# ceselder/pacman-marl-2025

Measured on AMD Instinct MI355X. Metric: env-steps/s (4-agent smallCapture), higher is better.
Workload: dtype u32; 1 GPU; smallCapture.lay 2v2, 16384 envs/GPU, gymPacMan tick (self_play), length 300, auto-reset, uniform random actions (Philox seed 1234), 4 observations/env-tick; envs_per_gpu=16384, layout=smallCapture, obs_dtype=float32, obs_bytes_per_elem=4, parallelism=env-sharded x1, no data-path collective

## Files before the change

### pacman-marl-2025_amd/csrc/pmx_actor.hip

```cpp
#pragma clang fp contract(fast)
#include <hip/hip_runtime.h>
#include <hip/hip_bf16.h>
#include <stdint.h>

#include "../../include/pmx.h"

namespace {

typedef __attribute__((ext_vector_type(8))) short bf16x8;
typedef __attribute__((ext_vector_type(4))) short bf16x4;
typedef __attribute__((ext_vector_type(4))) float f32x4;
typedef __attribute__((ext_vector_type(2))) float f32x2;
typedef __attribute__((ext_vector_type(2))) __bf16 bf16x2_t;

constexpr int NLAYER = 8;
constexpr int GUARD = 1;
constexpr int FRAG_PER_LAYER = 2 * 9 * 64 * 8;
constexpr size_t PACK_FWD = 0;
constexpr size_t PACK_BWD = PACK_FWD + (size_t)NLAYER * FRAG_PER_LAYER * 2;
constexpr size_t PACK_BIAS = PACK_BWD + (size_t)NLAYER * FRAG_PER_LAYER * 2;
constexpr size_t PACK_GNW = PACK_BIAS + NLAYER * 32 * 4;
constexpr size_t PACK_GNB = PACK_GNW + NLAYER * 32 * 4;
constexpr size_t PACK_BYTES = PACK_GNB + NLAYER * 32 * 4;
static_assert(PACK_BYTES == PMX_ACTOR_PACK_BYTES, "include/pmx.h and pmx_actor.hip disagree on the pack size");
constexpr int GRAD_W = 0;
constexpr int GRAD_B = GRAD_W + NLAYER * 36 * 256;
constexpr int GRAD_GNW = GRAD_B + NLAYER * 32;
constexpr int GRAD_GNB = GRAD_GNW + NLAYER * 32;
constexpr int GRAD_FLOATS = GRAD_GNB + NLAYER * 32;
constexpr int W_PART_ROWS = 128;
static_assert(GRAD_FLOATS == PMX_ACTOR_GRAD_FLOATS, "include/pmx.h and pmx_actor.hip disagree on the gradient size");

__host__ __device__ constexpr int map_positions(int nt, int wp) { return GUARD + wp + 32 * ((nt + 1) / 2) + wp + 3; }

__device__ __forceinline__ int map_off(int pos, int chunk) { return pos * 64 + (chunk << 4); }

__device__ __forceinline__ uint32_t pack2(float a, float b)
{
    f32x2 f = {a, b};
    return __builtin_bit_cast(uint32_t, __builtin_convertvector(f, bf16x2_t));
}
__device__ __forceinline__ float lo_f(uint32_t u) { return __uint_as_float(u << 16); }
__device__ __forceinline__ float hi_f(uint32_t u) { return __uint_as_float(u & 0xFFFF0000u); }

__device__ __forceinline__ f32x2 fma2(f32x2 a, f32x2 b, f32x2 c) { return __builtin_elementwise_fma(a, b, c); }
__device__ __forceinline__ f32x2 splat2(float v) { return f32x2{v, v}; }
__device__ __forceinline__ f32x2 unpack2(uint32_t u) { return f32x2{lo_f(u), hi_f(u)}; }
__device__ __forceinline__ f32x2 phi_cdf2(f32x2 z, f32x2 &e)
{
    const f32x2 den = {fmaf(0.3275911f * 0.70710678118654752f, fabsf(z.x), 1.0f), fmaf(0.3275911f * 0.70710678118654752f, fabsf(z.y), 1.0f)};
    const f32x2 t = {__builtin_amdgcn_rcpf(den.x), __builtin_amdgcn_rcpf(den.y)};
    f32x2 poly = fma2(t, splat2(0.5f * 1.061405429f), splat2(0.5f * -1.453152027f));
    poly = fma2(poly, t, splat2(0.5f * 1.421413741f));
    poly = fma2(poly, t, splat2(0.5f * -0.284496736f));
    poly = fma2(poly, t, splat2(0.5f * 0.254829592f));
    poly *= t;
    const f32x2 arg = (z * z) * splat2(-0.5f * 1.4426950408889634f);
    e = f32x2{__builtin_amdgcn_exp2f(arg.x), __builtin_amdgcn_exp2f(arg.y)};
    const f32x2 half_tail = poly * e, rest = splat2(1.0f) - half_tail;
    return f32x2{z.x >= 0.0f ? rest.x : half_tail.x, z.y >= 0.0f ? rest.y : half_tail.y};
}
__device__ __forceinline__ uint2 gelu_quad(uint2 h2, uint2 r2, float mean, float rstd, const float (&gw)[4], const float (&gb)[4], float vm)
{
    f32x2 v[2];
#pragma unroll
    for (int k = 0; k < 2; ++k) {
        const f32x2 hv = unpack2(k ? h2.y : h2.x), rv = unpack2(k ? r2.y : r2.x);
        const f32x2 z = rv + fma2((hv - splat2(mean)) * splat2(rstd), f32x2{gw[2 * k], gw[2 * k + 1]}, f32x2{gb[2 * k], gb[2 * k + 1]});
        f32x2 e;
        v[k] = z * phi_cdf2(z, e) * splat2(vm);
    }
    return uint2{pack2(v[0].x, v[0].y), pack2(v[1].x, v[1].y)};
}
__device__ __forceinline__ uint2 dgelu_quad(uint2 dy, uint2 h2, uint2 x2, float rstd, float nmr, const f32x2 (&gw2)[2], const f32x2 (&gb2)[2],
                                            f32x2 (&dgw2)[2], f32x2 (&dgb2)[2])
{
    f32x2 xh[2], dzf[2];
#pragma unroll
    for (int k = 0; k < 2; ++k) {
        const f32x2 hv = unpack2(k ? h2.y : h2.x), xv = unpack2(k ? x2.y : x2.x), d = unpack2(k ? dy.y : dy.x);
        xh[k] = fma2(hv, splat2(rstd), splat2(nmr));
        const f32x2 z = xv + fma2(xh[k], gw2[k], gb2[k]);
        f32x2 e;
        const f32x2 phi = phi_cdf2(z, e);
        dzf[k] = d * fma2(z * splat2(0.3989422804014327f), e, phi);
    }
    uint2 dzq = {pack2(dzf[0].x, dzf[0].y), pack2(dzf[1].x, dzf[1].y)};
    asm volatile("" : "+v"(dzq.x), "+v"(dzq.y));
#pragma unroll
    for (int k = 0; k < 2; ++k) {
        const f32x2 dzr = unpack2(k ? dzq.y : dzq.x);
        dgb2[k] += dzr;
        dgw2[k] = fma2(dzr, xh[k], dgw2[k]);
    }
    return dzq;
}

template <typename T> __device__ __forceinline__ float in_to_f(T v);
template <> __device__ __forceinline__ float in_to_f<uint8_t>(uint8_t v) { return (float)v; }
template <> __device__ __forceinline__ float in_to_f<float>(float v) { return v; }
template <> __device__ __forceinline__ float in_to_f<__hip_bfloat16>(__hip_bfloat16 v) { return __bfloat162float(v); }

__device__ __forceinline__ void wave_lds_fence()
{
    __builtin_amdgcn_fence(__ATOMIC_ACQ_REL, "wavefront");
    __builtin_amdgcn_wave_barrier();
}

template <int CTRL> __device__ __forceinline__ float dpp_f(float v)
{
    return __builtin_bit_cast(float, __builtin_amdgcn_update_dpp(0, __builtin_bit_cast(int, v), CTRL, 0xF, 0xF, true));
}
__device__ __forceinline__ float row16_sum(float v)
{
    v += dpp_f<0xB1>(v);
    v += dpp_f<0x4E>(v);
    v += dpp_f<0x141>(v);
    v += dpp_f<0x140>(v);
    return v;
}
__device__ __forceinline__ float group_sum(float v)
{
    v = row16_sum(v);
    float a = v, b = v;
    asm volatile("s_nop 1\n\tv_permlane16_swap_b32 %0, %1" : "+v"(a), "+v"(b));
    return a + b;
}
__device__ __forceinline__ float pos_sum(float v) { return row16_sum(v); }

struct Geom {
    int H, W, WP, HW, MP;
};

template <typename IN_T>
__device__ __forceinline__ void load_obs(const IN_T *__restrict__ obs, char *map, const Geom &G, int lane)
{
    for (int i = lane; i < G.HW; i += 64) {
        const int row = i / G.W, col = i - row * G.W;
        const int pos = (row + 1) * G.WP + col + 1 + GUARD;
        float v[8];
#pragma unroll
        for (int c = 0; c < 8; ++c) v[c] = in_to_f<IN_T>(obs[c * G.HW + i]);
        uint4 w = {pack2(v[0], v[1]), pack2(v[2], v[3]), pack2(v[4], v[5]), pack2(v[6], v[7])};
        *reinterpret_cast<uint4 *>(map + map_off(pos, 0)) = w;
        const uint4 z = {0, 0, 0, 0};
#pragma unroll
        for (int ch = 1; ch < 4; ++ch) *reinterpret_cast<uint4 *>(map + map_off(pos, ch)) = z;
    }
}

__device__ __forceinline__ void load_frags(bf16x8 (&A)[2][9], const short *__restrict__ frag, int lane)
{
#pragma unroll
    for (int m = 0; m < 2; ++m)
#pragma unroll
        for (int k = 0; k < 9; ++k) A[m][k] = *reinterpret_cast<const bf16x8 *>(frag + ((m * 9 + k) * 64 + lane) * 8);
}

__device__ __forceinline__ void conv_tile(const char *lane_base, const bf16x8 (&A)[2][9], int centre, int wp64, f32x4 &a0, f32x4 &a1)
{
    a0 = f32x4{0.f, 0.f, 0.f, 0.f};
    a1 = f32x4{0.f, 0.f, 0.f, 0.f};
#pragma unroll
    for (int ky = 0; ky < 3; ++ky) {
        const char *row = lane_base + (centre + (ky - 1) * wp64 - 64);
#pragma unroll
        for (int kx = 0; kx < 3; ++kx) {
            const bf16x8 b = *reinterpret_cast<const bf16x8 *>(row + kx * 64);
            a0 = __builtin_amdgcn_mfma_f32_16x16x32_bf16(A[0][ky * 3 + kx], b, a0, 0, 0, 0);
            a1 = __builtin_amdgcn_mfma_f32_16x16x32_bf16(A[1][ky * 3 + kx], b, a1, 0, 0, 0);
        }
    }
}

__device__ __forceinline__ size_t dump_index(size_t sample, int NT, int t, int m, int lane) { return ((sample * NT + t) * 2 + m) * 64 + lane; }

template <int NT, typename IN_T, bool SAVE>
__global__ __launch_bounds__(256, 2) void pmx_actor_fwd_kernel(const IN_T *__restrict__ obs, const char *__restrict__ pack,
                                                              uint2 *__restrict__ feat, uint2 *__restrict__ hsave,
                                                              uint2 *__restrict__ ysave, float *__restrict__ stats,
                                                              uint2 *__restrict__ rtmp, int B, int H, int W, float eps)
{
    extern __shared__ __attribute__((aligned(16))) char smem[];
    const int lane = threadIdx.x & 63, wave = threadIdx.x >> 6;
    const int p = lane & 15, g = lane >> 4;
    Geom G;
    G.H = H, G.W = W, G.WP = W + 2, G.HW = H * W, G.MP = map_positions(NT, W + 2);
    char *map = smem + (size_t)wave * G.MP * 64;
    for (int i = lane; i < G.MP * 4; i += 64) reinterpret_cast<uint4 *>(map)[i] = uint4{0, 0, 0, 0};
    __shared__ int cell_tab[NT * 16];
    for (int i = threadIdx.x; i < NT * 16; i += 256) {
        const int q = G.WP + i, row = q / G.WP, col = q - row * G.WP;
        cell_tab[i] = (col >= 1 && col <= W && row <= H) ? (row - 1) * W + (col - 1) : -1;
    }
    __syncthreads();
    uint32_t vmask = 0;
#pragma unroll
    for (int t = 0; t < NT; ++t) {
        const int q = G.WP + 16 * t + p, row = q / G.WP, col = q - row * G.WP;
        if (col >= 1 && col <= W && row <= H) vmask |= 1u << t;
    }
    const short *fw = reinterpret_cast<const short *>(pack + PACK_FWD);
    const float *biasp = reinterpret_cast<const float *>(pack + PACK_BIAS);
    const float *gnwp = reinterpret_cast<const float *>(pack + PACK_GNW);
    const float *gnbp = reinterpret_cast<const float *>(pack + PACK_GNB);
    const float inv_n = 1.0f / (float)(8 * G.HW);

    for (int s = blockIdx.x * 4 + wave; s < B; s += gridDim.x * 4) {
        wave_lds_fence();
        load_obs<IN_T>(obs + (size_t)s * 8 * G.HW, map, G, lane);
        wave_lds_fence();
        const short *fws = fw;
        asm volatile("" : "+s"(fws));
        bf16x8 A[2][9];
        load_frags(A, fws, lane);
#pragma unroll 1
        for (int li = 0; li < NLAYER; ++li) {
            int l = li;
            asm volatile("" : "+s"(l));
            const bool has_gn = l >= 2;
            const bool res_on = l >= 3 && (l & 1);
            int WPv = G.WP, pq = p + GUARD;
            uint32_t vmk = vmask;
            asm volatile("" : "+s"(WPv));
            asm volatile("" : "+v"(pq), "+v"(vmk));
            uint2 *ydst = SAVE ? ysave + dump_index((size_t)l * B + s, NT, 0, 0, lane)
                               : rtmp + dump_index((size_t)blockIdx.x * 4 + wave, NT, 0, 0, lane);
            const uint2 *rsrc = SAVE ? ysave + dump_index((size_t)(l >= 2 ? l - 2 : 0) * B + s, NT, 0, 0, lane) : ydst;
            const bool write_y = SAVE || (l & 1);
            float bias[2][4];
#pragma unroll
            for (int m = 0; m < 2; ++m)
#pragma unroll
                for (int r = 0; r < 4; ++r) bias[m][r] = biasp[l * 32 + 16 * m + 4 * g + r];
            uint2 hp[NT][2];
            float s1[2] = {0.f, 0.f}, s2[2] = {0.f, 0.f};
            const char *rbase = map + pq * 64 + g * 16;
            char *wbase = map + pq * 64 + g * 8;
#pragma unroll
            for (int t = 0; t < NT; ++t) {
                f32x4 a[2];
                conv_tile(rbase, A, (WPv + 16 * t) * 64, WPv * 64, a[0], a[1]);
                const float vm = ((vmk >> t) & 1) ? 1.0f : 0.0f;
#pragma unroll
                for (int m = 0; m < 2; ++m) {
                    float v[4];
#pragma unroll
                    for (int r = 0; r < 4; ++r) v[r] = (a[m][r] + bias[m][r]) * vm;
                    uint2 h2 = {pack2(v[0], v[1]), pack2(v[2], v[3])};
                    asm volatile("" : "+v"(h2.x), "+v"(h2.y));
                    hp[t][m] = h2;
                    const float h0 = lo_f(h2.x), h1 = hi_f(h2.x), h2f = lo_f(h2.y), h3 = hi_f(h2.y);
                    s1[m] += (h0 + h1) + (h2f + h3);
                    s2[m] += fmaf(h0, h0, h1 * h1) + fmaf(h2f, h2f, h3 * h3);
                    if (SAVE) hsave[dump_index((size_t)l * B + s, NT, t, m, lane)] = h2;
                }
                __builtin_amdgcn_sched_barrier(0);
            }
            load_frags(A, fws + (size_t)(l + 1 < NLAYER ? l + 1 : l) * FRAG_PER_LAYER, lane);
            constexpr int RD = 2;
            float gw[2][4], gb[2][4];
            uint2 rres[NT][2];
#pragma unroll
            for (int t = 0; t < NT; ++t) rres[t][0] = rres[t][1] = uint2{0u, 0u};
            if (res_on) {
#pragma unroll
                for (int t = 0; t < RD; ++t)
#pragma unroll
                    for (int m = 0; m < 2; ++m) rres[t][m] = rsrc[(t * 2 + m) * 64];
            }
            float mean[2], rstd[2];
#pragma unroll
            for (int m = 0; m < 2; ++m) {
                const float a1 = group_sum(s1[m]) * inv_n, a2 = group_sum(s2[m]) * inv_n;
                mean[m] = has_gn ? a1 : 0.0f;
                rstd[m] = has_gn ? __builtin_amdgcn_rsqf(fmaxf(a2 - a1 * a1, 0.0f) + eps) : 1.0f;
            }
            if (SAVE && p == 0 && (g & 1) == 0) {
#pragma unroll
                for (int m = 0; m < 2; ++m) {
                    float *st = stats + (((size_t)l * B + s) * 4 + 2 * m + (g >> 1)) * 2;
                    st[0] = mean[m], st[1] = rstd[m];
                }
            }
#pragma unroll
            for (int m = 0; m < 2; ++m)
#pragma unroll
                for (int r = 0; r < 4; ++r) gw[m][r] = gnwp[l * 32 + 16 * m + 4 * g + r], gb[m][r] = gnbp[l * 32 + 16 * m + 4 * g + r];
            wave_lds_fence();
#pragma unroll
            for (int t = 0; t < NT; ++t) {
                const float vm = ((vmk >> t) & 1) ? 1.0f : 0.0f;
                if (t + RD < NT && res_on) {
#pragma unroll
                    for (int m = 0; m < 2; ++m) rres[t + RD][m] = rsrc[((t + RD) * 2 + m) * 64];
                }
#pragma unroll
                for (int m = 0; m < 2; ++m) {
                    const uint2 y2 = gelu_quad(hp[t][m], rres[t][m], mean[m], rstd[m], gw[m], gb[m], vm);
                    *reinterpret_cast<uint2 *>(wbase + (WPv + 16 * t) * 64 + m * 32) = y2;
                    if (write_y) ydst[(t * 2 + m) * 64] = y2;
                    if (l == NLAYER - 1) {
                        const int ci = cell_tab[16 * t + p];
                        if (ci >= 0) feat[((size_t)s * G.HW + ci) * 8 + 4 * m + g] = y2;
                    }
                    __builtin_amdgcn_sched_barrier(0);
// ... 410 lines not shown
#pragma unroll
        for (int w = 0; w < 4; ++w) v += reinterpret_cast<const float *>(smem + (size_t)w * (G.MP * 64 + NLAYER * 96 * 4) + (size_t)G.MP * 64)[i];
        accpart[(size_t)blockIdx.x * (NLAYER * 96) + i] = v;
    }
}

template <int NT, int WS>
__global__ __launch_bounds__(256, 2) void pmx_actor_bwd_data_split_kernel(const char *__restrict__ pack, const uint2 *__restrict__ dfeat,
                                                                         const uint2 *__restrict__ hsave, const uint2 *__restrict__ ysave,
                                                                         const float *__restrict__ stats, bf16x8 *__restrict__ dasave,
                                                                         uint2 *__restrict__ sktmp, float *__restrict__ accpart, int B,
                                                                         int H, int W)
{
    constexpr int NTW = (NT + WS - 1) / WS, SPB = 4 / WS, KS = (NT + 1) / 2;
    constexpr bool XG_LATE = NT > 16;
    extern __shared__ __attribute__((aligned(16))) char smem[];
    const int lane = threadIdx.x & 63, wave = threadIdx.x >> 6;
    const int p = lane & 15, g = lane >> 4;
    Geom G;
    G.H = H, G.W = W, G.WP = W + 2, G.HW = H * W, G.MP = map_positions(NT, W + 2);
    const int sub = __builtin_amdgcn_readfirstlane(wave / WS), wq = __builtin_amdgcn_readfirstlane(wave % WS);
    char *map = smem + (size_t)sub * G.MP * 64;
    float *acc = reinterpret_cast<float *>(smem + (size_t)SPB * G.MP * 64) + wave * (NLAYER * 96);
    float *xs = reinterpret_cast<float *>(smem + (size_t)SPB * G.MP * 64) + 4 * (NLAYER * 96) + sub * (WS * 8);
    for (int i = threadIdx.x; i < SPB * G.MP * 4; i += 256) reinterpret_cast<uint4 *>(smem)[i] = uint4{0, 0, 0, 0};
    for (int i = lane; i < NLAYER * 96; i += 64) acc[i] = 0.0f;
    const int t0 = __builtin_amdgcn_readfirstlane(wq * NTW);
    uint32_t vmask = 0;
#pragma unroll
    for (int tl = 0; tl < NTW; ++tl) {
        const int q = G.WP + 16 * (t0 + tl) + p, row = q / G.WP, col = q - row * G.WP;
        if (t0 + tl < NT && col >= 1 && col <= W && row <= H) vmask |= 1u << tl;
    }
    const short *bw = reinterpret_cast<const short *>(pack + PACK_BWD);
    const float *gnwp = reinterpret_cast<const float *>(pack + PACK_GNW);
    const float *gnbp = reinterpret_cast<const float *>(pack + PACK_GNB);
    const float inv_n = 1.0f / (float)(8 * G.HW);
    const int tr_row = (lane & 15) >> 2, tr_pc = lane & 3;

    for (int s0 = blockIdx.x * SPB; s0 < B; s0 += gridDim.x * SPB) {
        const bool live = s0 + sub < B;
        const int s = live ? s0 + sub : B - 1;
        uint2 dv[NTW][2];
        uint2 *skp = sktmp + dump_index((size_t)blockIdx.x * SPB + sub, NT, 0, 0, lane);
        {
            int WPo = G.WP;
            asm volatile("" : "+s"(WPo));
#pragma unroll
            for (int tl = 0; tl < NTW; ++tl) {
                const int q = WPo + 16 * (t0 + tl) + p, row = q / WPo, col = q - row * WPo;
                const bool valid = (vmask >> tl) & 1;
#pragma unroll
                for (int m = 0; m < 2; ++m) {
                    dv[tl][m] = uint2{0, 0};
                    if (valid) dv[tl][m] = dfeat[((size_t)s * G.HW + (row - 1) * W + (col - 1)) * 8 + 4 * m + g];
                }
            }
        }
        uint2 hp[NTW][2], xg[NTW][2];
        float gw[2][4], gb[2][4], mean[2], rstd[2], nmr[2];
        auto load_layer_inputs = [&](int ln) {
            const bool res_n = ln >= 3 && (ln & 1);
            const int lres = ln >= 2 ? ln - 2 : 0;
#pragma unroll
            for (int m = 0; m < 2; ++m) {
#pragma unroll
                for (int r = 0; r < 4; ++r) gw[m][r] = gnwp[ln * 32 + 16 * m + 4 * g + r], gb[m][r] = gnbp[ln * 32 + 16 * m + 4 * g + r];
                const float *st = stats + (((size_t)ln * B + s) * 4 + 2 * m + (g >> 1)) * 2;
                mean[m] = st[0], rstd[m] = st[1];
                nmr[m] = -mean[m] * rstd[m];
            }
#pragma unroll
            for (int tl = 0; tl < NTW; ++tl)
#pragma unroll
                for (int m = 0; m < 2; ++m) {
                    hp[tl][m] = uint2{0u, 0u};
                    if (!XG_LATE) xg[tl][m] = uint2{0u, 0u};
                    if (t0 + tl < NT) {
                        hp[tl][m] = hsave[dump_index((size_t)ln * B + s, NT, t0 + tl, m, lane)];
                        if (!XG_LATE && res_n) xg[tl][m] = ysave[dump_index((size_t)lres * B + s, NT, t0 + tl, m, lane)];
                    }
                }
        };
        load_layer_inputs(NLAYER - 1);
#pragma unroll 1
        for (int li = NLAYER - 1; li >= 0; --li) {
            int l = __builtin_amdgcn_readfirstlane(li);
            asm volatile("" : "+s"(l));
            const bool has_gn = l >= 2, has_res = l >= 3 && (l & 1), adds_skip = l >= 2 && !(l & 1);
            const float gn_on = has_gn ? 1.0f : 0.0f;
            int WPv = G.WP, pq = p + GUARD;
            uint32_t vmk = vmask;
            asm volatile("" : "+s"(WPv));
            asm volatile("" : "+v"(pq), "+v"(vmk));
            if (XG_LATE) {
#pragma unroll
                for (int tl = 0; tl < NTW; ++tl)
#pragma unroll
                    for (int m = 0; m < 2; ++m) {
                        xg[tl][m] = uint2{0u, 0u};
                        if (has_res && t0 + tl < NT) xg[tl][m] = ysave[dump_index((size_t)(l - 2) * B + s, NT, t0 + tl, m, lane)];
                    }
            }
            float S1[2], S2[2];
            float dgw[2][4], dgb[2][4];
            f32x2 dgw2[2][2], dgb2[2][2], gw2[2][2], gb2[2][2];
#pragma unroll
            for (int m = 0; m < 2; ++m)
#pragma unroll
                for (int k = 0; k < 2; ++k) {
                    dgw2[m][k] = dgb2[m][k] = f32x2{0.0f, 0.0f};
                    gw2[m][k] = f32x2{gw[m][2 * k], gw[m][2 * k + 1]}, gb2[m][k] = f32x2{gb[m][2 * k], gb[m][2 * k + 1]};
                }
#pragma unroll
            for (int tl = 0; tl < NTW; ++tl) {
                if (t0 + tl < NT) {
#pragma unroll
                    for (int m = 0; m < 2; ++m) {
                        dv[tl][m] = dgelu_quad(dv[tl][m], hp[tl][m], xg[tl][m], rstd[m], nmr[m], gw2[m], gb2[m], dgw2[m], dgb2[m]);
                        __builtin_amdgcn_sched_barrier(0);
                    }
                }
            }
#pragma unroll
            for (int m = 0; m < 2; ++m)
#pragma unroll
                for (int k = 0; k < 2; ++k)
                    dgw[m][2 * k] = dgw2[m][k].x, dgw[m][2 * k + 1] = dgw2[m][k].y, dgb[m][2 * k] = dgb2[m][k].x, dgb[m][2 * k + 1] = dgb2[m][k].y;
            if (has_res) {
#pragma unroll
                for (int tl = 0; tl < NTW; ++tl)
                    if (t0 + tl < NT) {
#pragma unroll
                        for (int m = 0; m < 2; ++m) skp[((t0 + tl) * 2 + m) * 64] = dv[tl][m];
                    }
            }
#pragma unroll
            for (int m = 0; m < 2; ++m) {
                float t1 = 0.f, t2 = 0.f;
#pragma unroll
                for (int r = 0; r < 4; ++r) t1 = fmaf(gw[m][r], dgb[m][r], t1), t2 = fmaf(gw[m][r], dgw[m][r], t2);
                const float a1 = group_sum(t1), a2 = group_sum(t2);
                if (p == 0 && (g & 1) == 0) {
                    xs[(wq * 4 + 2 * m + (g >> 1)) * 2] = a1;
                    xs[(wq * 4 + 2 * m + (g >> 1)) * 2 + 1] = a2;
                }
            }
            const short *bws = bw + (size_t)l * FRAG_PER_LAYER;
            asm volatile("" : "+s"(bws));
            bf16x8 A[2][9];
            load_frags(A, bws, lane);
            __syncthreads();
#pragma unroll
            for (int m = 0; m < 2; ++m) {
                const int grp = 2 * m + (g >> 1);
                float a1 = 0.f, a2 = 0.f;
#pragma unroll
                for (int w = 0; w < WS; ++w) { a1 += xs[(w * 4 + grp) * 2]; a2 += xs[(w * 4 + grp) * 2 + 1]; }
                S1[m] = a1 * inv_n * gn_on, S2[m] = a2 * inv_n * gn_on;
            }
            float Ad[2][4], K2[2], K3[2];
#pragma unroll
            for (int m = 0; m < 2; ++m) {
                K2[m] = -rstd[m] * rstd[m] * S2[m];
                K3[m] = -mean[m] * K2[m] - rstd[m] * S1[m];
#pragma unroll
                for (int r = 0; r < 4; ++r) Ad[m][r] = rstd[m] * gw[m][r];
            }
            float dbias[2][4];
#pragma unroll
            for (int m = 0; m < 2; ++m)
#pragma unroll
                for (int r = 0; r < 4; ++r) dbias[m][r] = 0.0f;
            char *wbase = map + pq * 64 + g * 8;
#pragma unroll
            for (int tl = 0; tl < NTW; ++tl) {
                const int t = t0 + tl;
                if (t < NT) {
                    const float vm = ((vmk >> tl) & 1) ? 1.0f : 0.0f;
#pragma unroll
                    for (int m = 0; m < 2; ++m) {
                        const uint2 h2 = hp[tl][m];
                        const float hv[4] = {lo_f(h2.x), hi_f(h2.x), lo_f(h2.y), hi_f(h2.y)};
                        const float dzr[4] = {lo_f(dv[tl][m].x), hi_f(dv[tl][m].x), lo_f(dv[tl][m].y), hi_f(dv[tl][m].y)};
                        float dh[4];
#pragma unroll
                        for (int r = 0; r < 4; ++r) dh[r] = vm * fmaf(Ad[m][r], dzr[r], fmaf(hv[r], K2[m], K3[m]));
                        const uint2 d2 = {pack2(dh[0], dh[1]), pack2(dh[2], dh[3])};
                        dbias[m][0] += lo_f(d2.x), dbias[m][1] += hi_f(d2.x), dbias[m][2] += lo_f(d2.y), dbias[m][3] += hi_f(d2.y);
                        *reinterpret_cast<uint2 *>(wbase + (WPv + 16 * t) * 64 + m * 32) = d2;
                    }
                }
                __builtin_amdgcn_sched_barrier(0);
            }
            uint2 skip[NTW][2];
#pragma unroll
            for (int tl = 0; tl < NTW; ++tl) {
                skip[tl][0] = skip[tl][1] = uint2{0u, 0u};
                if (adds_skip && t0 + tl < NT) {
#pragma unroll
                    for (int m = 0; m < 2; ++m) skip[tl][m] = skp[((t0 + tl) * 2 + m) * 64];
                }
            }
            load_layer_inputs(l > 0 ? l - 1 : 0);
            if (live) {
#pragma unroll
                for (int m = 0; m < 2; ++m)
#pragma unroll
                    for (int r = 0; r < 4; ++r) {
                        const float b = pos_sum(dbias[m][r]), w = pos_sum(dgw[m][r]), c = pos_sum(dgb[m][r]);
                        if (p == 0) {
                            float *a3 = acc + l * 96 + 16 * m + 4 * g + r;
                            a3[0] += b, a3[32] += w, a3[64] += c;
                        }
                    }
            }
            __syncthreads();
            {
                bf16x8 *dst = dasave + (((size_t)l * B + s) * KS * 2) * 64 + lane;
                const char *tbase = map + (8 * g + tr_row + GUARD) * 64 + tr_pc * 8;
#pragma unroll 1
                for (int ks = wq; ks < KS; ks += WS) {
#pragma unroll
                    for (int mo = 0; mo < 2; ++mo) {
                        const char *o0 = tbase + (WPv + 32 * ks) * 64 + mo * 32;
                        const bf16x4 lo = __builtin_amdgcn_ds_read_tr16_b64_v4i16((bf16x4 __attribute__((address_space(3))) *)(o0));
                        const bf16x4 hi = __builtin_amdgcn_ds_read_tr16_b64_v4i16((bf16x4 __attribute__((address_space(3))) *)(o0 + 256));
                        dst[(ks * 2 + mo) * 64] = bf16x8{lo[0], lo[1], lo[2], lo[3], hi[0], hi[1], hi[2], hi[3]};
                    }
                }
            }
            if (l > 0) {
#pragma unroll
                for (int tl = 0; tl < NTW; ++tl) {
                    const int t = t0 + tl;
                    if (t < NT) {
                        f32x4 a[2];
                        conv_tile(map + pq * 64 + g * 16, A, (WPv + 16 * t) * 64, WPv * 64, a[0], a[1]);
                        const float vm = ((vmk >> tl) & 1) ? 1.0f : 0.0f;
#pragma unroll
                        for (int m = 0; m < 2; ++m) {
                            const uint32_t sx = skip[tl][m].x, sy = skip[tl][m].y;
                            const float v0 = (lo_f(sx) + a[m][0]) * vm, v1 = (hi_f(sx) + a[m][1]) * vm;
                            const float v2 = (lo_f(sy) + a[m][2]) * vm, v3 = (hi_f(sy) + a[m][3]) * vm;
                            uint2 nx = {pack2(v0, v1), pack2(v2, v3)};
                            asm volatile("" : "+v"(nx.x), "+v"(nx.y));
                            dv[tl][m] = nx;
                        }
                    }
                    __builtin_amdgcn_sched_barrier(0);
                }
            }
        }
        __syncthreads();
    }
    __syncthreads();
    for (int i = threadIdx.x; i < NLAYER * 96; i += 256) {
        const float *a0 = reinterpret_cast<const float *>(smem + (size_t)SPB * G.MP * 64);
        accpart[(size_t)blockIdx.x * (NLAYER * 96) + i] = (a0[i] + a0[NLAYER * 96 + i]) + (a0[2 * NLAYER * 96 + i] + a0[3 * NLAYER * 96 + i]);
    }
}

__global__ __launch_bounds__(256) void pmx_actor_sum_acc_kernel(const float *__restrict__ accpart, int n_rows, float *__restrict__ grad)
{
    __shared__ float part[8][33];
    const int c = threadIdx.x & 31, sl = threadIdx.x >> 5;
    const int i = blockIdx.x * 32 + c;
    float acc[4] = {0.f, 0.f, 0.f, 0.f};
    int r = sl;
    for (; r + 24 < n_rows; r += 32) {
#pragma unroll
        for (int k = 0; k < 4; ++k) acc[k] += accpart[(size_t)(r + 8 * k) * (NLAYER * 96) + i];
    }
    for (; r < n_rows; r += 8) acc[0] += accpart[(size_t)r * (NLAYER * 96) + i];
    part[sl][c] = (acc[0] + acc[1]) + (acc[2] + acc[3]);
    __syncthreads();
    if (sl == 0) {
        float t = 0.f;
#pragma unroll
        for (int k = 0; k < 8; ++k) t += part[k][c];
        const int l = i / 96, j = i - l * 96, kind = j >> 5, ch = j & 31;
        grad[(kind == 0 ? GRAD_B : kind == 1 ? GRAD_GNW : GRAD_GNB) + l * 32 + ch] = t;
    }
}

__global__ __launch_bounds__(256) void pmx_actor_sum_w_kernel(const float *__restrict__ wpart, int n_rows, float *__restrict__ grad)
{
    __shared__ float part[8][33];
    const int c = threadIdx.x & 31, sl = threadIdx.x >> 5;
    const int i = blockIdx.x * 32 + c;
    constexpr size_t ROW = (size_t)NLAYER * 36 * 256;
    float acc = 0.f;
    for (int r = sl; r < n_rows; r += 8) acc += wpart[(size_t)r * ROW + i];
    part[sl][c] = acc;
    __syncthreads();
    if (sl == 0) {
        float t = 0.f;
#pragma unroll
        for (int k = 0; k < 8; ++k) t += part[k][c];
        grad[GRAD_W + i] = t;
    }
}

template <int NT, typename IN_T>
__global__ __launch_bounds__(256, 2) void pmx_actor_bwd_weight_kernel(const IN_T *__restrict__ obs, const uint2 *__restrict__ ysave,
                                                                     const bf16x8 *__restrict__ dasave, float *__restrict__ grad,
                                                                     int B, int H, int W, int per_wave)
{
    extern __shared__ __attribute__((aligned(16))) char smem[];
    const int lane = threadIdx.x & 63, wave = threadIdx.x >> 6;
    const int p = lane & 15, g = lane >> 4;
    const int l = blockIdx.y;
    Geom G;
    G.H = H, G.W = W, G.WP = W + 2, G.HW = H * W, G.MP = map_positions(NT, W + 2);
    constexpr int KS = (NT + 1) / 2;
    char *mapB = smem + (size_t)wave * G.MP * 64;
    for (int i = lane; i < G.MP * 4; i += 64) reinterpret_cast<uint4 *>(mapB)[i] = uint4{0, 0, 0, 0};
    const int tr_row = (lane & 15) >> 2, tr_pc = lane & 3;
    f32x4 accw[36];
#pragma unroll
    for (int i = 0; i < 36; ++i) accw[i] = f32x4{0.f, 0.f, 0.f, 0.f};
    const int s_begin = (blockIdx.x * 4 + wave) * per_wave;
    const int s_end = s_begin + per_wave < B ? s_begin + per_wave : B;
    for (int s = s_begin; s < s_end; ++s) {
        int WPv = G.WP, pq = p + GUARD;
        asm volatile("" : "+s"(WPv));
        asm volatile("" : "+v"(pq));
        wave_lds_fence();
        if (l == 0) {
            load_obs<IN_T>(obs + (size_t)s * 8 * G.HW, mapB, G, lane);
        } else {
            uint2 xin[NT][2];
#pragma unroll
            for (int t = 0; t < NT; ++t)
#pragma unroll
                for (int m = 0; m < 2; ++m) xin[t][m] = ysave[dump_index((size_t)(l - 1) * B + s, NT, t, m, lane)];
#pragma unroll
            for (int t = 0; t < NT; ++t)
#pragma unroll
                for (int m = 0; m < 2; ++m)
                    *reinterpret_cast<uint2 *>(mapB + pq * 64 + g * 8 + (WPv + 16 * t) * 64 + m * 32) = xin[t][m];
        }
        wave_lds_fence();
        const bf16x8 *asrc = dasave + (((size_t)l * B + s) * KS * 2) * 64 + lane;
#pragma unroll 1
        for (int ks = 0; ks < KS; ++ks) {
            const bf16x8 Ad0 = asrc[(ks * 2 + 0) * 64], Ad1 = asrc[(ks * 2 + 1) * 64];
            const char *tbase = mapB + (8 * g + tr_row + GUARD) * 64 + tr_pc * 8 + (WPv + 32 * ks) * 64;
#pragma unroll
            for (int ky = 0; ky < 3; ++ky)
#pragma unroll
                for (int kx = 0; kx < 3; ++kx) {
                    const char *tx = tbase + ((ky - 1) * WPv + (kx - 1)) * 64;
#pragma unroll
                    for (int ni = 0; ni < 2; ++ni) {
                        const bf16x4 lo = __builtin_amdgcn_ds_read_tr16_b64_v4i16((bf16x4 __attribute__((address_space(3))) *)(tx + ni * 32));
                        const bf16x4 hi = __builtin_amdgcn_ds_read_tr16_b64_v4i16((bf16x4 __attribute__((address_space(3))) *)(tx + ni * 32 + 256));
                        const bf16x8 Bx = bf16x8{lo[0], lo[1], lo[2], lo[3], hi[0], hi[1], hi[2], hi[3]};
                        accw[(0 * 2 + ni) * 9 + ky * 3 + kx] = __builtin_amdgcn_mfma_f32_16x16x32_bf16(Ad0, Bx, accw[(0 * 2 + ni) * 9 + ky * 3 + kx], 0, 0, 0);
                        accw[(1 * 2 + ni) * 9 + ky * 3 + kx] = __builtin_amdgcn_mfma_f32_16x16x32_bf16(Ad1, Bx, accw[(1 * 2 + ni) * 9 + ky * 3 + kx], 0, 0, 0);
                    }
                }
        }
    }
    __syncthreads();
    float *red = reinterpret_cast<float *>(smem);
    constexpr int PER_ROUND = 9;
#pragma unroll
    for (int round = 0; round < 4; ++round) {
#pragma unroll
        for (int i = 0; i < PER_ROUND; ++i)
            *reinterpret_cast<f32x4 *>(red + ((size_t)(wave * PER_ROUND + i) * 64 + lane) * 4) = accw[round * PER_ROUND + i];
        __syncthreads();
        for (int i = threadIdx.x; i < PER_ROUND * 64; i += 256) {
            f32x4 v = *reinterpret_cast<const f32x4 *>(red + (size_t)i * 4);
#pragma unroll
            for (int w = 1; w < 4; ++w) {
                const f32x4 u = *reinterpret_cast<const f32x4 *>(red + ((size_t)w * PER_ROUND * 64 + i) * 4);
                v[0] += u[0], v[1] += u[1], v[2] += u[2], v[3] += u[3];
            }
            float *dst = grad + ((size_t)blockIdx.x * NLAYER * 36 + (size_t)l * 36 + round * PER_ROUND) * 256 + (size_t)i * 4;
            *reinterpret_cast<f32x4 *>(dst) = v;
        }
        __syncthreads();
    }
}

template <int NT, typename IN_T>
__global__ __launch_bounds__(256, 2) void pmx_actor_bwd_weight_split_kernel(const IN_T *__restrict__ obs, const uint2 *__restrict__ ysave,
                                                                           const bf16x8 *__restrict__ dasave, float *__restrict__ wpart,
                                                                           int B, int H, int W, int per_pair)
{
    constexpr int KS = (NT + 1) / 2, NTH = (NT + 1) / 2;
    extern __shared__ __attribute__((aligned(16))) char smem[];
    const int lane = threadIdx.x & 63, wave = threadIdx.x >> 6;
    const int p = lane & 15, g = lane >> 4;
    const int l = blockIdx.y;
    const int sub = __builtin_amdgcn_readfirstlane(wave >> 1), ni = __builtin_amdgcn_readfirstlane(wave & 1);
    Geom G;
    G.H = H, G.W = W, G.WP = W + 2, G.HW = H * W, G.MP = map_positions(NT, W + 2);
    char *mapB = smem + (size_t)sub * G.MP * 64;
    for (int i = threadIdx.x; i < 2 * G.MP * 4; i += 256) reinterpret_cast<uint4 *>(smem)[i] = uint4{0, 0, 0, 0};
    const int tr_row = (lane & 15) >> 2, tr_pc = lane & 3;
    f32x4 accw[18];
#pragma unroll
    for (int i = 0; i < 18; ++i) accw[i] = f32x4{0.f, 0.f, 0.f, 0.f};
    const int pair = blockIdx.x * 2 + sub;
    const int s_begin = pair * per_pair;
    uint2 xin[NTH][2];
    auto fetch = [&](int s) {
#pragma unroll
        for (int tl = 0; tl < NTH; ++tl)
#pragma unroll
            for (int m = 0; m < 2; ++m) {
                const int t = ni * NTH + tl;
                xin[tl][m] = uint2{0u, 0u};
                if (t < NT) xin[tl][m] = ysave[dump_index((size_t)(l - 1) * B + s, NT, t, m, lane)];
            }
    };
    if (l > 0 && s_begin < B) fetch(s_begin);
    for (int i = 0; i < per_pair; ++i) {
        const int s = s_begin + i;
        const bool live = s < B;
        int WPv = G.WP, pq = p + GUARD;
        asm volatile("" : "+s"(WPv));
        asm volatile("" : "+v"(pq));
        __syncthreads();
        if (live) {
            if (l == 0) {
                load_obs_block<IN_T>(obs + (size_t)s * 8 * G.HW, mapB, G, ni * 64 + lane, 128);
            } else {
#pragma unroll
                for (int tl = 0; tl < NTH; ++tl) {
                    const int t = ni * NTH + tl;
                    if (t < NT) {
#pragma unroll
                        for (int m = 0; m < 2; ++m)
                            *reinterpret_cast<uint2 *>(mapB + pq * 64 + g * 8 + (WPv + 16 * t) * 64 + m * 32) = xin[tl][m];
                    }
                }
            }
        }
        __syncthreads();
        if (l > 0 && i + 1 < per_pair && s + 1 < B) fetch(s + 1);
        if (live) {
            const bf16x8 *asrc = dasave + (((size_t)l * B + s) * KS * 2) * 64 + lane;
            bf16x8 An0 = asrc[0], An1 = asrc[64];
#pragma unroll 2
            for (int ks = 0; ks < KS; ++ks) {
                const bf16x8 Ad0 = An0, Ad1 = An1;
                if (ks + 1 < KS) { An0 = asrc[((ks + 1) * 2 + 0) * 64]; An1 = asrc[((ks + 1) * 2 + 1) * 64]; }
                const char *tbase = mapB + (8 * g + tr_row + GUARD) * 64 + tr_pc * 8 + (WPv + 32 * ks) * 64 + ni * 32;
#pragma unroll
                for (int ky = 0; ky < 3; ++ky)
#pragma unroll
                    for (int kx = 0; kx < 3; ++kx) {
                        const char *tx = tbase + ((ky - 1) * WPv + (kx - 1)) * 64;
                        const bf16x4 lo = __builtin_amdgcn_ds_read_tr16_b64_v4i16((bf16x4 __attribute__((address_space(3))) *)(tx));
                        const bf16x4 hi = __builtin_amdgcn_ds_read_tr16_b64_v4i16((bf16x4 __attribute__((address_space(3))) *)(tx + 256));
                        const bf16x8 Bx = bf16x8{lo[0], lo[1], lo[2], lo[3], hi[0], hi[1], hi[2], hi[3]};
                        accw[ky * 3 + kx] = __builtin_amdgcn_mfma_f32_16x16x32_bf16(Ad0, Bx, accw[ky * 3 + kx], 0, 0, 0);
                        accw[9 + ky * 3 + kx] = __builtin_amdgcn_mfma_f32_16x16x32_bf16(Ad1, Bx, accw[9 + ky * 3 + kx], 0, 0, 0);
                    }
            }
        }
    }
    float *dst = wpart + ((size_t)pair * NLAYER * 36 + (size_t)l * 36) * 256 + (size_t)lane * 4;
#pragma unroll
    for (int mo = 0; mo < 2; ++mo)
#pragma unroll
        for (int k = 0; k < 9; ++k) *reinterpret_cast<f32x4 *>(dst + (size_t)((mo * 2 + ni) * 9 + k) * 256) = accw[mo * 9 + k];
}

struct PackArgs {
    const float *w[NLAYER], *b[NLAYER], *gw[NLAYER], *gb[NLAYER];
    int cin[NLAYER], cout[NLAYER];
};

__global__ __launch_bounds__(256) void pmx_actor_pack_kernel(PackArgs a, char *__restrict__ pack)
{
    const int l = blockIdx.y;
    short *fw = reinterpret_cast<short *>(pack + PACK_FWD) + (size_t)l * FRAG_PER_LAYER;
    short *bw = reinterpret_cast<short *>(pack + PACK_BWD) + (size_t)l * FRAG_PER_LAYER;
    const int cin = a.cin[l], cout = a.cout[l];
    for (int i = blockIdx.x * 256 + threadIdx.x; i < FRAG_PER_LAYER; i += gridDim.x * 256) {
        const int j = i & 7, lane = (i >> 3) & 63, k = (i >> 9) % 9, m = i / (512 * 9);
        const int row = 16 * m + (lane & 15), kk = 8 * (lane >> 4) + j;
        float vf = 0.f, vb = 0.f;
        if (row < cout && kk < cin) vf = a.w[l][((size_t)row * cin + kk) * 9 + k];
        if (row < cin && kk < cout) vb = a.w[l][((size_t)kk * cin + row) * 9 + (8 - k)];
        fw[i] = (short)(pack2(vf, 0.f) & 0xFFFF);
        bw[i] = (short)(pack2(vb, 0.f) & 0xFFFF);
    }
    if (blockIdx.x == 0 && threadIdx.x < 32) {
        const int c = threadIdx.x;
        reinterpret_cast<float *>(pack + PACK_BIAS)[l * 32 + c] = c < cout ? a.b[l][c] : 0.f;
        reinterpret_cast<float *>(pack + PACK_GNW)[l * 32 + c] = a.gw[l] ? a.gw[l][c] : 1.f;
        reinterpret_cast<float *>(pack + PACK_GNB)[l * 32 + c] = a.gb[l] ? a.gb[l][c] : 0.f;
    }
}

struct UnpackArgs {
    float *w[NLAYER], *b[NLAYER], *gw[NLAYER], *gb[NLAYER];
    int cin[NLAYER], cout[NLAYER];
};

__global__ __launch_bounds__(256) void pmx_actor_unpack_kernel(UnpackArgs a, const float *__restrict__ grad)
{
    const int l = blockIdx.y;
    const int cin = a.cin[l], cout = a.cout[l];
    for (int i = blockIdx.x * 256 + threadIdx.x; i < 36 * 256; i += gridDim.x * 256) {
        const int r = i & 3, lane = (i >> 2) & 63, tile = i >> 8;
        const int k = tile % 9, ni = (tile / 9) & 1, mo = tile / 18;
        const int co = 16 * mo + 4 * (lane >> 4) + r, ci = 16 * ni + (lane & 15);
        if (co < cout && ci < cin) a.w[l][((size_t)co * cin + ci) * 9 + k] = grad[GRAD_W + (size_t)l * 36 * 256 + i];
    }
    if (blockIdx.x == 0 && threadIdx.x < 32) {
        const int c = threadIdx.x;
        if (c < cout) a.b[l][c] = grad[GRAD_B + l * 32 + c];
        if (a.gw[l]) a.gw[l][c] = grad[GRAD_GNW + l * 32 + c];
        if (a.gb[l]) a.gb[l][c] = grad[GRAD_GNB + l * 32 + c];
    }
}

int tiles_for(int H, int W) { return (H * (W + 2) + 15) / 16; }

}

static const int kCin[NLAYER] = {8, 16, 32, 32, 32, 32, 32, 32};
static const int kCout[NLAYER] = {16, 32, 32, 32, 32, 32, 32, 32};

static bool tiles_supported(int nt) { return nt == 10 || nt == 11 || nt == 28; }
constexpr bool large_board(int nt) { return nt > 16; }

extern "C" int pmx_actor_supported(int32_t H, int32_t W)
{
    if (H < 1 || W < 1 || H > PMX_MAX_DIM || W > PMX_MAX_DIM) return 0;
    return tiles_supported(tiles_for(H, W)) ? 1 : 0;
}

extern "C" int pmx_actor_sizes(int32_t H, int32_t W, int64_t B, int64_t *save_bytes, int64_t *scratch_bytes, int64_t *infer_scratch_bytes)
{
    if (!pmx_actor_supported(H, W) || B < 0) return PMX_ERR_UNSUPPORTED;
    const int64_t dump = (int64_t)tiles_for(H, W) * 1024;
    if (save_bytes) *save_bytes = B * (8 * dump + 8 * dump + 8 * 4 * 2 * 4);
    const int64_t infer = 2048 * dump;
    if (infer_scratch_bytes) *infer_scratch_bytes = infer;
    if (scratch_bytes)
        *scratch_bytes = B * 8 * (int64_t)((tiles_for(H, W) + 1) / 2) * 2048 + infer + 1024 * 768 * 4 + (int64_t)W_PART_ROWS * NLAYER * 36 * 256 * 4;
    return PMX_OK;
}

extern "C" int pmx_actor_pack(const pmx_actor_params *p, void *pack_dev, void *stream)
{
    if (!p || !pack_dev) return PMX_ERR_INVALID;
    PackArgs a;
    for (int l = 0; l < NLAYER; ++l) {
        a.w[l] = p->conv_w[l], a.b[l] = p->conv_b[l];
        a.gw[l] = l >= 2 ? p->gn_w[l - 2] : nullptr, a.gb[l] = l >= 2 ? p->gn_b[l - 2] : nullptr;
        a.cin[l] = kCin[l], a.cout[l] = kCout[l];
        if (!a.w[l] || !a.b[l] || (l >= 2 && (!a.gw[l] || !a.gb[l]))) return PMX_ERR_INVALID;
    }
    hipLaunchKernelGGL(pmx_actor_pack_kernel, dim3(9, NLAYER), dim3(256), 0, reinterpret_cast<hipStream_t>(stream), a,
                       reinterpret_cast<char *>(pack_dev));
    return hipGetLastError() == hipSuccess ? PMX_OK : PMX_ERR_HIP;
}

extern "C" int pmx_actor_unpack_grads(const float *grad_dev, const pmx_actor_params *out, void *stream)
{
    if (!grad_dev || !out) return PMX_ERR_INVALID;
    UnpackArgs a;
    for (int l = 0; l < NLAYER; ++l) {
        a.w[l] = const_cast<float *>(out->conv_w[l]), a.b[l] = const_cast<float *>(out->conv_b[l]);
        a.gw[l] = l >= 2 ? const_cast<float *>(out->gn_w[l - 2]) : nullptr;
        a.gb[l] = l >= 2 ? const_cast<float *>(out->gn_b[l - 2]) : nullptr;
        a.cin[l] = kCin[l], a.cout[l] = kCout[l];
        if (!a.w[l] || !a.b[l] || (l >= 2 && (!a.gw[l] || !a.gb[l]))) return PMX_ERR_INVALID;
    }
    hipLaunchKernelGGL(pmx_actor_unpack_kernel, dim3(9, NLAYER), dim3(256), 0, reinterpret_cast<hipStream_t>(stream), a, grad_dev);
    return hipGetLastError() == hipSuccess ? PMX_OK : PMX_ERR_HIP;
}

namespace {

template <typename K> int allow_lds(K kernel, size_t lds)
{
    if (lds <= 65536) return PMX_OK;
    struct Key { const void *fn; int dev; };
    static Key done[256];
    static int n_done = 0;
    int dev = 0;
    if (hipGetDevice(&dev) != hipSuccess) return PMX_ERR_HIP;
    const void *fn = reinterpret_cast<const void *>(kernel);
    for (int i = 0; i < n_done; ++i)
        if (done[i].fn == fn && done[i].dev == dev) return PMX_OK;
    if (hipFuncSetAttribute(fn, hipFuncAttributeMaxDynamicSharedMemorySize, 160 * 1024) != hipSuccess) return PMX_ERR_HIP;
    if (n_done < 256) done[n_done++] = Key{fn, dev};
    return PMX_OK;
}

int grid_for(int64_t B, int blocks_per_cu)
{
    int dev = 0, cus = 256;
    if (hipGetDevice(&dev) != hipSuccess || hipDeviceGetAttribute(&cus, hipDeviceAttributeMultiprocessorCount, dev) != hipSuccess) cus = 256;
    const int64_t want = (B + 3) / 4;
    const int64_t cap = (int64_t)cus * blocks_per_cu;
    return (int)(want < cap ? want : cap);
}

constexpr int64_t SPLIT_MAX_BATCH = 1536;
constexpr int64_t SPLIT_BWD_MAX_BATCH = 512;
constexpr int64_t BWD_TWO_WAVE_MIN = 4096;

constexpr int split_waves(int64_t B) { return B <= 512 ? 4 : 2; }

template <int NT, typename IN_T>
int launch_fwd(const void *obs, const void *pack, void *feat, void *save, void *scratch, int64_t B, int H, int W, hipStream_t st)
{
    const int64_t dump = (int64_t)NT * 128;
    uint2 *hs = reinterpret_cast<uint2 *>(save), *ys = hs ? hs + 8 * B * dump : nullptr;
    float *stt = hs ? reinterpret_cast<float *>(ys + 8 * B * dump) : nullptr;
    uint2 *rtmp = reinterpret_cast<uint2 *>(scratch);
    if (!save && !rtmp) return PMX_ERR_INVALID;
    if (large_board(NT) || B <= SPLIT_MAX_BATCH) {
        const int ws = large_board(NT) ? 4 : split_waves(B);
        const int spb = 4 / ws;
        const size_t lds_s = (size_t)spb * map_positions(NT, W + 2) * 64 + (size_t)spb * ws * 8 * sizeof(float);
        int64_t g64 = (B + spb - 1) / spb;
        if (g64 * spb > 2048) g64 = 2048 / spb;
        const unsigned grid = (unsigned)g64;
#define PMX_FWD_SPLIT(SAVEV, WSV)                                                                                           \
    do {                                                                                                                    \
        int rc = allow_lds(pmx_actor_fwd_split_kernel<NT, IN_T, SAVEV, WSV>, lds_s);                                        \
        if (rc) return rc;                                                                                                  \
        hipLaunchKernelGGL((pmx_actor_fwd_split_kernel<NT, IN_T, SAVEV, WSV>), dim3(grid), dim3(256), lds_s, st, (const IN_T *)obs, \
                           (const char *)pack, (uint2 *)feat, hs, ys, stt, rtmp, (int)B, H, W, 1e-5f);                       \
    } while (0)
        if constexpr (large_board(NT)) {
            if (save) PMX_FWD_SPLIT(true, 4); else PMX_FWD_SPLIT(false, 4);
        } else {
            if (save) { if (ws == 2) PMX_FWD_SPLIT(true, 2); else PMX_FWD_SPLIT(true, 4); }
            else { if (ws == 2) PMX_FWD_SPLIT(false, 2); else PMX_FWD_SPLIT(false, 4); }
        }
#undef PMX_FWD_SPLIT
        return hipGetLastError() == hipSuccess ? PMX_OK : PMX_ERR_HIP;
    }
    if constexpr (!large_board(NT)) {
        const size_t lds = (size_t)4 * map_positions(NT, W + 2) * 64;
        if (save) {
            int rc = allow_lds(pmx_actor_fwd_kernel<NT, IN_T, true>, lds);
            if (rc) return rc;
            hipLaunchKernelGGL((pmx_actor_fwd_kernel<NT, IN_T, true>), dim3(grid_for(B, 2)), dim3(256), lds, st, (const IN_T *)obs,
                               (const char *)pack, (uint2 *)feat, hs, ys, stt, rtmp, (int)B, H, W, 1e-5f);
        } else {
            int rc = allow_lds(pmx_actor_fwd_kernel<NT, IN_T, false>, lds);
            if (rc) return rc;
            hipLaunchKernelGGL((pmx_actor_fwd_kernel<NT, IN_T, false>), dim3(grid_for(B, 2)), dim3(256), lds, st, (const IN_T *)obs,
                               (const char *)pack, (uint2 *)feat, hs, ys, stt, rtmp, (int)B, H, W, 1e-5f);
        }
    }
    return hipGetLastError() == hipSuccess ? PMX_OK : PMX_ERR_HIP;
}

template <int NT, typename IN_T>
int launch_bwd(const void *obs, const void *pack, const void *save, const void *dfeat, void *scratch, float *grad, int64_t B,
               int H, int W, hipStream_t st)
{
// ... 389 lines not shown
```

Before: 325.7 million env-steps/s.

## Software-pipeline weight-gradient kernel loads and specialize first layer

Restructures the backward weight-gradient kernel into a templated per-sample routine that prefetches the next sample's inputs and activation-gradient fragments while computing the current one, using a three-slot register ring for the gradient fragments. Layer 0 gets its own specialization that loads observations straight into registers and skips the MFMAs and fragment loads for the half of the channel blocks it does not need. The aim is to hide global-load latency behind MFMA work and drop wasted layer-0 compute, at the cost of more register pressure and scheduling barriers.

```diff
diff --git a/pacman-marl-2025_amd/csrc/pmx_actor.hip b/pacman-marl-2025_amd/csrc/pmx_actor.hip
--- a/pacman-marl-2025_amd/csrc/pmx_actor.hip
+++ b/pacman-marl-2025_amd/csrc/pmx_actor.hip
@@ -2,6 +2,7 @@
 #include <hip/hip_runtime.h>
 #include <hip/hip_bf16.h>
 #include <stdint.h>
+#include <type_traits>
 
 #include "../../include/pmx.h"
 
@@ -1018,67 +1019,145 @@
     }
 }
 
+
+template <int NT, typename IN_T, bool L0>
+__device__ __forceinline__ void wgrad_samples(f32x4 (&accw)[36], const IN_T *__restrict__ obs, const uint2 *__restrict__ ysave,
+                                              const bf16x8 *__restrict__ dasave, char *mapB, const Geom &G, int l, int B, int s_begin,
+                                              int s_end, int lane)
+{
+    constexpr int KS = (NT + 1) / 2;
+    constexpr int OI = (NT * 16 + 63) / 64;
+    const int p = lane & 15, g = lane >> 4;
+    const int tr_row = (lane & 15) >> 2, tr_pc = lane & 3;
+    if (s_begin >= s_end) return;
+    uint2 xin[L0 ? 1 : NT][2];
+    IN_T ob[L0 ? OI : 1][8];
+    int opos[L0 ? OI : 1];
+    if constexpr (L0) {
+#pragma unroll
+        for (int k = 0; k < OI; ++k) {
+            const int i = lane + 64 * k, row = i / G.W, col = i - row * G.W;
+            opos[k] = map_off((row + 1) * G.WP + col + 1 + GUARD, 0);
+        }
+    }
+    auto fetch = [&](int s) {
+        if constexpr (L0) {
+            const IN_T *src = obs + (size_t)s * 8 * G.HW;
+#pragma unroll
+            for (int k = 0; k < OI; ++k)
+                if (lane + 64 * k < G.HW) {
+#pragma unroll
+                    for (int c = 0; c < 8; ++c) ob[k][c] = src[c * G.HW + lane + 64 * k];
+                }
+        } else {
+#pragma unroll
+            for (int t = 0; t < NT; ++t)
+#pragma unroll
+                for (int m = 0; m < 2; ++m) xin[t][m] = ysave[dump_index((size_t)(l - 1) * B + s, NT, t, m, lane)];
+        }
+    };
+    auto put = [&](int WPv, int pq) {
+        if constexpr (L0) {
+#pragma unroll
+            for (int k = 0; k < OI; ++k)
+                if (lane + 64 * k < G.HW) {
+                    float v[8];
+#pragma unroll
+                    for (int c = 0; c < 8; ++c) v[c] = in_to_f<IN_T>(ob[k][c]);
+                    *reinterpret_cast<uint4 *>(mapB + opos[k]) = uint4{pack2(v[0], v[1]), pack2(v[2], v[3]), pack2(v[4], v[5]), pack2(v[6], v[7])};
+                }
+        } else {
+#pragma unroll
+            for (int t = 0; t < NT; ++t)
+#pragma unroll
+                for (int m = 0; m < 2; ++m)
+                    *reinterpret_cast<uint2 *>(mapB + pq * 64 + g * 8 + (WPv + 16 * t) * 64 + m * 32) = xin[t][m];
+        }
+    };
+    auto frag = [&](int s, int ks) { return dasave + (((size_t)l * B + s) * KS + ks) * 128 + lane; };
+    constexpr int KV = 6;
+    static_assert(KS <= KV && KS >= KV - 1, "the ring counts six key-pair blocks per sample");
+    auto sample = [&](int s, auto more_c, bf16x8 (&R0)[3], bf16x8 (&R1)[3]) {
+        constexpr bool MORE = decltype(more_c)::value;
+        int WPv = G.WP, pq = p + GUARD;
+        asm volatile("" : "+s"(WPv));
+        asm volatile("" : "+v"(pq));
+        wave_lds_fence();
+        put(WPv, pq);
+        wave_lds_fence();
+        asm volatile("" : "+v"(R0[0]));
+        if constexpr (!L0) asm volatile("" : "+v"(R1[0]));
+        if constexpr (MORE) fetch(s + 1);
+#pragma unroll 1
+        for (int tr = 0; tr < KV / 3; ++tr) {
+#pragma unroll
+            for (int j = 0; j < 3; ++j) {
+                const int ks = 3 * tr + j, v = ks + 2;
+                if (v < KS) {
+                    const bf16x8 *nx = frag(s, v);
+                    R0[(j + 2) % 3] = nx[0];
+                    if constexpr (!L0) R1[(j + 2) % 3] = nx[64];
+                } else if (MORE && v >= KV) {
+                    const bf16x8 *nx = frag(s + 1, v - KV);
+                    R0[(j + 2) % 3] = nx[0];
+                    if constexpr (!L0) R1[(j + 2) % 3] = nx[64];
+                }
+                __builtin_amdgcn_sched_barrier(0);
+                if (ks < KS) {
+                    const bf16x8 Ad0 = R0[j], Ad1 = R1[j];
+                    const char *tbase = mapB + (8 * g + tr_row + GUARD) * 64 + tr_pc * 8 + (WPv + 32 * ks) * 64;
+#pragma unroll
+                    for (int ky = 0; ky < 3; ++ky) {
+#pragma unroll
+                        for (int kx = 0; kx < 3; ++kx) {
+                            const char *tx = tbase + ((ky - 1) * WPv + (kx - 1)) * 64;
+#pragma unroll
+                            for (int ni = 0; ni < (L0 ? 1 : 2); ++ni) {
+                                const bf16x4 lo = __builtin_amdgcn_ds_read_tr16_b64_v4i16((bf16x4 __attribute__((address_space(3))) *)(tx + ni * 32));
+                                const bf16x4 hi = __builtin_amdgcn_ds_read_tr16_b64_v4i16((bf16x4 __attribute__((address_space(3))) *)(tx + ni * 32 + 256));
+                                const bf16x8 Bx = bf16x8{lo[0], lo[1], lo[2], lo[3], hi[0], hi[1], hi[2], hi[3]};
+                                accw[(0 * 2 + ni) * 9 + ky * 3 + kx] = __builtin_amdgcn_mfma_f32_16x16x32_bf16(Ad0, Bx, accw[(0 * 2 + ni) * 9 + ky * 3 + kx], 0, 0, 0);
+                                if constexpr (!L0)
+                                    accw[(1 * 2 + ni) * 9 + ky * 3 + kx] = __builtin_amdgcn_mfma_f32_16x16x32_bf16(Ad1, Bx, accw[(1 * 2 + ni) * 9 + ky * 3 + kx], 0, 0, 0);
+                            }
+                        }
+                    }
+                }
+                __builtin_amdgcn_sched_barrier(0);
+            }
+        }
+    };
+    fetch(s_begin);
+    bf16x8 R0[3], R1[3];
+#pragma unroll
+    for (int k = 0; k < 2; ++k) R0[k] = frag(s_begin, k)[0], R1[k] = frag(s_begin, L0 ? 0 : k)[L0 ? 0 : 64];
+    R0[2] = R0[0], R1[2] = R1[0];
+    int s = s_begin;
+    for (; s + 1 < s_end; ++s) sample(s, std::true_type{}, R0, R1);
+    sample(s, std::false_type{}, R0, R1);
+}
+
 template <int NT, typename IN_T>
 __global__ __launch_bounds__(256, 2) void pmx_actor_bwd_weight_kernel(const IN_T *__restrict__ obs, const uint2 *__restrict__ ysave,
                                                                      const bf16x8 *__restrict__ dasave, float *__restrict__ grad,
                                                                      int B, int H, int W, int per_wave)
 {
     extern __shared__ __attribute__((aligned(16))) char smem[];
-    const int lane = threadIdx.x & 63, wave = threadIdx.x >> 6;
-    const int p = lane & 15, g = lane >> 4;
+    const int lane = threadIdx.x & 63, wave = __builtin_amdgcn_readfirstlane(threadIdx.x >> 6);
     const int l = blockIdx.y;
     Geom G;
     G.H = H, G.W = W, G.WP = W + 2, G.HW = H * W, G.MP = map_positions(NT, W + 2);
-    constexpr int KS = (NT + 1) / 2;
     char *mapB = smem + (size_t)wave * G.MP * 64;
     for (int i = lane; i < G.MP * 4; i += 64) reinterpret_cast<uint4 *>(mapB)[i] = uint4{0, 0, 0, 0};
-    const int tr_row = (lane & 15) >> 2, tr_pc = lane & 3;
     f32x4 accw[36];
 #pragma unroll
     for (int i = 0; i < 36; ++i) accw[i] = f32x4{0.f, 0.f, 0.f, 0.f};
     const int s_begin = (blockIdx.x * 4 + wave) * per_wave;
     const int s_end = s_begin + per_wave < B ? s_begin + per_wave : B;
-    for (int s = s_begin; s < s_end; ++s) {
-        int WPv = G.WP, pq = p + GUARD;
-        asm volatile("" : "+s"(WPv));
-        asm volatile("" : "+v"(pq));
-        wave_lds_fence();
-        if (l == 0) {
-            load_obs<IN_T>(obs + (size_t)s * 8 * G.HW, mapB, G, lane);
-        } else {
-            uint2 xin[NT][2];
-#pragma unroll
-            for (int t = 0; t < NT; ++t)
-#pragma unroll
-                for (int m = 0; m < 2; ++m) xin[t][m] = ysave[dump_index((size_t)(l - 1) * B + s, NT, t, m, lane)];
-#pragma unroll
-            for (int t = 0; t < NT; ++t)
-#pragma unroll
-                for (int m = 0; m < 2; ++m)
-                    *reinterpret_cast<uint2 *>(mapB + pq * 64 + g * 8 + (WPv + 16 * t) * 64 + m * 32) = xin[t][m];
-        }
-        wave_lds_fence();
-        const bf16x8 *asrc = dasave + (((size_t)l * B + s) * KS * 2) * 64 + lane;
-#pragma unroll 1
-        for (int ks = 0; ks < KS; ++ks) {
-            const bf16x8 Ad0 = asrc[(ks * 2 + 0) * 64], Ad1 = asrc[(ks * 2 + 1) * 64];
-            const char *tbase = mapB + (8 * g + tr_row + GUARD) * 64 + tr_pc * 8 + (WPv + 32 * ks) * 64;
-#pragma unroll
-            for (int ky = 0; ky < 3; ++ky)
-#pragma unroll
-                for (int kx = 0; kx < 3; ++kx) {
-                    const char *tx = tbase + ((ky - 1) * WPv + (kx - 1)) * 64;
-#pragma unroll
-                    for (int ni = 0; ni < 2; ++ni) {
-                        const bf16x4 lo = __builtin_amdgcn_ds_read_tr16_b64_v4i16((bf16x4 __attribute__((address_space(3))) *)(tx + ni * 32));
-                        const bf16x4 hi = __builtin_amdgcn_ds_read_tr16_b64_v4i16((bf16x4 __attribute__((address_space(3))) *)(tx + ni * 32 + 256));
-                        const bf16x8 Bx = bf16x8{lo[0], lo[1], lo[2], lo[3], hi[0], hi[1], hi[2], hi[3]};
-                        accw[(0 * 2 + ni) * 9 + ky * 3 + kx] = __builtin_amdgcn_mfma_f32_16x16x32_bf16(Ad0, Bx, accw[(0 * 2 + ni) * 9 + ky * 3 + kx], 0, 0, 0);
-                        accw[(1 * 2 + ni) * 9 + ky * 3 + kx] = __builtin_amdgcn_mfma_f32_16x16x32_bf16(Ad1, Bx, accw[(1 * 2 + ni) * 9 + ky * 3 + kx], 0, 0, 0);
-                    }
-                }
-        }
-    }
+    if (l == 0)
+        wgrad_samples<NT, IN_T, true>(accw, obs, ysave, dasave, mapB, G, l, B, s_begin, s_end, lane);
+    else
+        wgrad_samples<NT, IN_T, false>(accw, obs, ysave, dasave, mapB, G, l, B, s_begin, s_end, lane);
     __syncthreads();
     float *red = reinterpret_cast<float *>(smem);
     constexpr int PER_ROUND = 9;
```

New measurement: 324.8 million env-steps/s. Within noise of the previous version (-0.3%).
